# foolwood/SiamMask

Hardware: AMD Instinct MI355X
Metric: frames/sec (255x255 search, 127x127 template) (higher is better)
Workload: dtype f16

## Files before the change

siammask_amd/csrc/conv_plan.h:

```cpp
#pragma once
#include <string>
#include <vector>

#include "smk_kernels.h"

struct Act {
    void *p = nullptr;
    int H = 0, W = 0, C = 0;
};

struct PackedConv {
    void *w = nullptr;
    void *w_halo = nullptr;
    void *w_frag = nullptr;
    void *w_frag_halo = nullptr;
    void *w_frag16 = nullptr;
    float *bias = nullptr;
    int N = 0;
    int rows = 0;
    int group_rows = 0;
    int groups = 1;
    int Ci = 0, k = 1, K = 0, Kpad = 0;
    int kw = 0;
    int alg_k = 0;
// ... 2 lines not shown
    bool x3 = false;
};

struct ConvOpt {
    int stride = 1, pad = 0, dil = 1, relu = 0;
    int stride_x = 0;
    const Act *res = nullptr;
    int res_mode = smk::RES_NONE;
    int res_coff = 0;
    int cin_off = 0;
    int cout_off = 0;
    int n_override = 0;
    int groups = 1;
    bool win = false;
    int Hl = 0, Wl = 0, org_y = 0, org_x = 0;
    const int *pos = nullptr;
    int pos_mul = 0, pos_add = 0;
    bool ups = false;
    float *nchw_out = nullptr;
    int algo_naive = 0;
    int tile_code = 0;
    int halo = 0;
    int wreg = 0;
};

inline int kdtype(int dtype) { return dtype == smk::DT_F16X3 ? smk::DT_F16 : dtype; }
inline const char *dtname(int dt) { return dt == smk::DT_F16 ? "f16" : "f32"; }

#pragma GCC visibility push(hidden)

enum ConvKernel { CK_NAIVE, CK_IGEMM, CK_HALO, CK_WREG, CK_PP };
struct ConvPlan {
    int kind = CK_IGEMM;
    smk::TileChoice tile{};
    int halo_bm = 0;
    int wreg = 0;
    int stages = 0;
};

extern const int WREG_TILE[9][2];

smk::TileChoice tile_from_code(int code, const smk::ConvParams &p, int dtype);
int halo_choice(const PackedConv &pc, const smk::ConvParams &p, const ConvOpt &o, int dtype);
int wreg_choice(const smk::ConvParams &p, const ConvOpt &o, int dtype, long ncu);
int wreg_stages(int ctx_dtype, int B);
int wreg_stages_from_code(int code);
// ... 28 lines not shown
```

siammask_amd/csrc/conv_wreg.hip:

```cpp
#include <hip/hip_runtime.h>
#include <type_traits>
#include "smk_kernels.h"

namespace smk {

#include "wreg_tile.inc"

template <int WK, int MODE> struct WregDepth {
    static constexpr int NSTAGE = MODE == 8 ? 2 * WK + 1 : MODE;
    static constexpr int WT = MODE == 8 ? 2 * WK : 2;
};

template <int FM, int WN, int WK, int MODE, int NPW>
__global__ __launch_bounds__((WN * WK + NPW) * 64, ((NPW == 2 && WregLds<FM, WregDepth<WK, MODE>::NSTAGE, WN * WK>::v <= 80 * 1024) ? 2 : 1))
void conv_wreg_kernel(const ConvBatch cb) {
    constexpr int NSTAGE = WregDepth<WK, MODE>::NSTAGE, WT = WregDepth<WK, MODE>::WT;
    int pi = 0;
#pragma unroll
    for (int i = 1; i < CONV_BATCH_MAX; ++i)
        if (i < cb.n && (int)blockIdx.x >= cb.start[i]) pi = i;
    const ConvParams &p = cb.p[pi];
    set_wave_prio(cb.p[0].wave_prio);
    const int wg_first = cb.start[pi], wg_count = cb.start[pi + 1] - cb.start[pi];
    constexpr int BM = 32 * FM, BN = 64 * WN;
    __shared__ __attribute__((aligned(16))) unsigned char smem[WregLds<FM, NSTAGE, WN * WK>::v];
    const int tilesN = (p.Nst + BN - 1) / BN;
    int t = (int)blockIdx.x - wg_first;
    if (p.xcd_mode != 0) {
        const int nblk = wg_count, q = nblk >> 3, r = nblk & 7;
        const int x = t & 7, j = t >> 3;
        t = x * q + (x < r ? x : r) + j;
    }
    const int tm = t / tilesN, tn = t - tm * tilesN;
    wreg_tile<FM, WN, WK, NSTAGE, 0, WT, NPW>(p, (int)blockIdx.z, tm * BM, p.M, tn * BN, smem);
}

#ifdef SMK_MEASURE
template <int FM, int WN, int WK, int ABL>
__global__ __launch_bounds__(512, 1)
void conv_wreg_ablate_kernel(const ConvBatch cb) {
    const ConvParams &p = cb.p[0];
    constexpr int BM = 32 * FM, BN = 64 * WN;
    __shared__ __attribute__((aligned(16))) unsigned char smem[WregLds<FM, 3>::v];
    const int tilesN = (p.Nst + BN - 1) / BN;
    const int t = (int)blockIdx.x;
    const int tm = t / tilesN, tn = t - tm * tilesN;
    wreg_tile<FM, WN, WK, 3, (ABL << 8), 2, 4>(p, 0, tm * BM, p.M, tn * BN, smem);
}
#endif

template <int FM, int WN, int WK>
static int launch_wreg_t(ConvBatch &cb, int stages, hipStream_t s) {
    constexpr int BM = 32 * FM, BN = 64 * WN;
    int total = 0, groups = 1;
    for (int i = 0; i < cb.n; ++i) {
        ConvParams &p = cb.p[i];
        cb.start[i] = total;
        total += ((p.M + BM - 1) / BM) * ((p.Nst + BN - 1) / BN);
        if (p.groups > groups) groups = p.groups;
        p.ksplit = 1;
        if (p.x3_ct > 0 && p.x3_in > 0) {
            p.Ci = p.x3_in * X3_PLANES;
            p.ci_shift = -1;
            for (int sh = 0; sh < 16; ++sh)
                if ((1 << sh) == p.Ci) p.ci_shift = sh;
            p.x3_in = 0;
        }
    }
    for (int i = cb.n; i <= CONV_BATCH_MAX; ++i) cb.start[i] = total;
    dim3 grid(total, 1, groups);
#ifdef SMK_MEASURE
    if constexpr ((WN == 2 && WK == 2) || (WN == 4 && WK == 1))
    if (g_tune.ablate && cb.n == 1 && groups == 1) {
        switch (g_tune.ablate) {
        case 1: hipLaunchKernelGGL((conv_wreg_ablate_kernel<FM, WN, WK, 1>), grid, dim3(512), 0, s, cb); break;
        case 2: hipLaunchKernelGGL((conv_wreg_ablate_kernel<FM, WN, WK, 2>), grid, dim3(512), 0, s, cb); break;
        case 3: hipLaunchKernelGGL((conv_wreg_ablate_kernel<FM, WN, WK, 3>), grid, dim3(512), 0, s, cb); break;
        case 4: hipLaunchKernelGGL((conv_wreg_ablate_kernel<FM, WN, WK, 4>), grid, dim3(512), 0, s, cb); break;
        case 7: hipLaunchKernelGGL((conv_wreg_ablate_kernel<FM, WN, WK, 7>), grid, dim3(512), 0, s, cb); break;
        case 8: hipLaunchKernelGGL((conv_wreg_ablate_kernel<FM, WN, WK, 8>), grid, dim3(512), 0, s, cb); break;
        case 16: hipLaunchKernelGGL((conv_wreg_ablate_kernel<FM, WN, WK, 16>), grid, dim3(512), 0, s, cb); break;
        case 32: hipLaunchKernelGGL((conv_wreg_ablate_kernel<FM, WN, WK, 32>), grid, dim3(512), 0, s, cb); break;
        case 64: hipLaunchKernelGGL((conv_wreg_ablate_kernel<FM, WN, WK, 64>), grid, dim3(512), 0, s, cb); break;
        case 11: hipLaunchKernelGGL((conv_wreg_ablate_kernel<FM, WN, WK, 11>), grid, dim3(512), 0, s, cb); break;
        case 27: hipLaunchKernelGGL((conv_wreg_ablate_kernel<FM, WN, WK, 27>), grid, dim3(512), 0, s, cb); break;
        default: hipLaunchKernelGGL((conv_wreg_ablate_kernel<FM, WN, WK, 23>), grid, dim3(512), 0, s, cb); break;
        }
        return hipGetLastError() == hipSuccess ? 0 : -4;
    }
#endif
    if (g_tune.npw == 4) {
#ifdef SMK_MEASURE
        if (stages == 8 && WK > 1) {
            hipLaunchKernelGGL((conv_wreg_kernel<FM, WN, WK, (WK > 1 ? 8 : 3), 4>), grid, dim3((WN * WK + 4) * 64), 0, s, cb);
            return hipGetLastError() == hipSuccess ? 0 : -4;
        }
        if (stages == 5 || stages == 6 || stages == 7) {
            if (stages == 5) hipLaunchKernelGGL((conv_wreg_kernel<FM, WN, WK, 5, 4>), grid, dim3((WN * WK + 4) * 64), 0, s, cb);
            else if (stages == 6) hipLaunchKernelGGL((conv_wreg_kernel<FM, WN, WK, 6, 4>), grid, dim3((WN * WK + 4) * 64), 0, s, cb);
            else hipLaunchKernelGGL((conv_wreg_kernel<FM, WN, WK, 7, 4>), grid, dim3((WN * WK + 4) * 64), 0, s, cb);
            return hipGetLastError() == hipSuccess ? 0 : -4;
        }
#endif
        if (stages == 4) hipLaunchKernelGGL((conv_wreg_kernel<FM, WN, WK, 4, 4>), grid, dim3((WN * WK + 4) * 64), 0, s, cb);
        else hipLaunchKernelGGL((conv_wreg_kernel<FM, WN, WK, 3, 4>), grid, dim3((WN * WK + 4) * 64), 0, s, cb);
    } else {
        if (stages == 4) hipLaunchKernelGGL((conv_wreg_kernel<FM, WN, WK, 4, 2>), grid, dim3((WN * WK + 2) * 64), 0, s, cb);
        else hipLaunchKernelGGL((conv_wreg_kernel<FM, WN, WK, 3, 2>), grid, dim3((WN * WK + 2) * 64), 0, s, cb);
    }
    return hipGetLastError() == hipSuccess ? 0 : -4;
}

bool conv_wreg_eligible(const ConvParams &p, int dtype) {
    return dtype == DT_F16 && p.out_mode == OUT_NHWC && p.wgt_frag != nullptr && p.buf_lds && (p.Kpad % 128) == 0 &&
           (p.groups <= 1 || (p.g_wgt_off % 32) == 0);
}

int launch_conv_wreg_batch(ConvBatch &cb, int bm, int bn, int stages, void *stream) {
    hipStream_t s = (hipStream_t)stream;
    if (cb.n < 1 || cb.n > CONV_BATCH_MAX) return -1;
    for (int i = 0; i < cb.n; ++i)
        if (!conv_wreg_eligible(cb.p[i], DT_F16) || (cb.p[i].groups > 1) != (cb.p[0].groups > 1)) return 1;
    if (bm == 32) {
        if (bn == 64) return launch_wreg_t<1, 1, 4>(cb, stages, s);
    } else if (bm == 64) {
        if (bn == 256) return launch_wreg_t<2, 4, 1>(cb, stages, s);
        if (bn == 128) return launch_wreg_t<2, 2, 2>(cb, stages, s);
        if (bn == 64) return launch_wreg_t<2, 1, 4>(cb, stages, s);
    } else if (bm == 96) {
        if (bn == 256) return launch_wreg_t<3, 4, 1>(cb, stages, s);
    } else if (bm == 128) {
        if (bn == 256) return launch_wreg_t<4, 4, 1>(cb, stages, s);
        if (bn == 128) return launch_wreg_t<4, 2, 2>(cb, stages, s);
        if (bn == 64) return launch_wreg_t<4, 1, 4>(cb, stages, s);
    }
    return 1;
}

// ... 2 lines not shown
```

siammask_amd/csrc/engine.cpp:

```cpp
#include <hip/hip_runtime_api.h>

#include <cmath>
#include <cstdarg>
#include <tuple>
#include <cstdio>
#include <cstdlib>
#include <cstring>
#include <functional>
#include <map>
#include <memory>
#include <string>
#include <vector>

#include "../../include/siammask_hip.h"
#include "../../include/siammask_hip_test.h"
#include "conv_plan.h"
#include "smk_kernels.h"
#include "tracker_state.h"
#include "vot_overlap.h"

using namespace smk;

static thread_local std::string g_err;

// ... 717 lines not shown
        if (!out) return fail(SMK_E_ARG, "conv without output");
        if (out->H != p.Ho || out->W != p.Wo)
            return fail(SMK_E_ARG, "internal: conv output %dx%d != buffer %dx%d", p.Ho, p.Wo, out->H, out->W);
        p.out = out->p;
        p.out_mode = OUT_NHWC;
        p.Cos = out->C;
        p.cout_off = o.cout_off;
        p.Nst = rup(p.N, 8);
        if (pc.x3) {
            p.x3_out = o.groups > 1 ? pc.group_rows : out->C / X3_PLANES;
            if (out->C % X3_PLANES || o.cout_off + (o.groups - 1) * X3_PLANES * pc.group_rows + p.x3_out + p.Nst > out->C)
                return fail(SMK_E_ARG, "internal: split conv output channels exceed buffer");
        } else if (o.cout_off + (o.groups - 1) * pc.group_rows + p.Nst > out->C)
            return fail(SMK_E_ARG, "internal: conv output channels exceed buffer");
    }
    p.xcd_mode = g_tune.xcd_mode;
    if (o.nchw_out && g_tune.nchw_tn_major && p.xcd_mode == 1 && p.M >= 20000 && (double)p.M * p.N * 4 >= 4.0e6) p.xcd_mode = 2;
    p.prio = g_tune.prio;
    p.wave_prio = env.wave_prio;
    {
        const double ib = (double)B * in.H * in.W * in.C * esize(env.dtype), wb = (double)pc.rows * pc.Kpad * esize(env.dtype);
        p.buf_lds = (g_tune.buf_lds && ib < 2.0e9 && wb < 2.0e9) ? 1 : 0;
        p.a_stage = g_tune.a_stage;
        p.res_nt = g_tune.res_nt;
        p.in_bytes = (unsigned)(ib < 4.0e9 ? ib : 0);
        p.w_bytes = (unsigned)(wb < 4.0e9 ? wb : 0);
    }
    p.nt_store = (g_tune.nt_store && o.nchw_out && (double)p.M * p.N * 4 >= 4.0e6) ? 1 : 0;
    p.ci_shift = -1;
    for (int sh = 0; sh < 16; ++sh)
        if ((1 << sh) == p.Ci) p.ci_shift = sh;
    p.kw_magic = 65536 / p.kw + 1;
    p.zero = env.device >= 0 ? zero_page() : nullptr;
    if (env.device >= 0 && !p.zero) return fail(SMK_E_HIP, "could not allocate the zero page");
    if (o.res) {
        p.res = o.res->p;
        p.res_Cs = o.res->C;
        p.res_coff = o.res_coff;
        p.res_mode = o.res_mode;
        if (pc.x3) p.x3_res = o.res->C / X3_PLANES;
    }
    p.ksplit = 1;
    p.ks_part = env.ks_part;
    p.ks_cnt = env.ks_cnt;
    p.ks_part_cap = env.ks_part ? KS_PART_FLOATS : 0;
    p.ks_cnt_cap = env.ks_cnt ? KS_CNT : 0;
// ... 423 lines not shown
                    paired = run_conv_pair(c, (id + "c3").c_str(), t2, out, o3, "adjust", se, oa0, B, s);
                    if (paired < 0) return paired;
                    if (paired == 0) adjust_done = true;
                }
            }
            if (paired == 1) CHK(run_conv(c, (id + "c3").c_str(), t2, &out, B, o3, s, &rec));
            cur = out;
            sp = so;
        }
    }
    ConvOpt oa;
    if (sp < 20) {
        Act zf = ACT(c, T_ZF, sp - 8, sp - 8);
        oa.win = true; oa.Hl = oa.Wl = sp - 8; oa.org_y = oa.org_x = 4;
        CHK(run_conv(c, "adjust", cur, &zf, B, oa, s, &rec));
    } else if (!adjust_done) {
        Act se = ACT(c, T_SEARCH, sp, sp);
        CHK(run_conv(c, "adjust", cur, &se, B, oa, s, &rec));
    }
    if (c->seq_on && search_nb > 0 && sp >= 20 && g_tune.seq_search && c->seq.rec.size() < (size_t)SEQ_MAX) {
        Act se = ACT(c, T_SEARCH, sp, sp);
        Act xs = ACT(c, T_XS, sp - 2, sp - 2);
        ConvOpt o; o.relu = 1; o.n_override = 256 * search_nb;
        CHK(run_conv(c, "conv_search", se, &xs, B, o, s, &rec));
        if (search_done) *search_done = true;
    }
    if (c->seq_on) CHK(seq_flush(c, rec, B, s));
    c->last_B = B; c->last_S = S;
    return 0;
}

static int seq_template(smk_ctx *c, StepRec &rec, const float *z, int B, hipStream_t s) {
    CHK(run_backbone(c, rec, z, B, 127, s));
    Act zf = ACT(c, T_ZF);
    Act zk = ACT(c, T_ZK);
    ConvOpt o; o.relu = 1;
    CHK(run_conv(c, "conv_kernel", zf, &zk, B, o, s));
    return 0;
}

static int mask_head_args(smk_ctx *c, float *mask, Act &h0, ConvOpt &om) {
    CHK(act(h0, c, T_HEAD0));
    om.nchw_out = mask;
    om.cin_off = branch_off(c, 2);
    return 0;
}

static int seq_track(smk_ctx *c, StepRec &rec, const float *x, int B, int flags, float *cls, float *loc, float *mask,
                     hipStream_t s, int phase = PH_ALL) {
    const bool x3 = c->dtype == DT_F16X3;
    const int nbt = nbranch(c);
    const int nb = (flags & SMK_TRACK_MASK) ? nbt : 2;
    bool search_done = false;
    CHK(run_backbone(c, rec, x, B, 255, s, phase, nb, &search_done));
    Act se = ACT(c, T_SEARCH);
    Act xs = ACT(c, T_XS);
    ConvOpt o; o.relu = 1; o.n_override = 256 * nb;
    if (!search_done) CHK(run_conv(c, "conv_search", se, &xs, B, o, s));
    if (rec.gate_late) {
        if (launch_pipe_gate(c->pipe_cnt, c->seq_err, c->seq_err_hdev, s, 0, nullptr, c->pipe_cnt + 8)) return fail(SMK_E_HIP, "pipe_gate launch failed");
        rec.has_seq = true;
    }
    Act zk = ACT(c, T_ZK);
    Act corr = ACT(c, T_CORR);
    Act h0 = ACT(c, T_HEAD0);
    const bool want_mask = (flags & SMK_TRACK_MASK) && !(flags & SMK_TRACK_NO_MASK_HEAD);
    bool fused_heads = false;
    if (c->dtype == DT_F16 && g_tune.corr_head) {
        auto ih = c->conv.find("head0"), ic = c->conv.find("cls3"), il = c->conv.find("loc3");
        if (ih != c->conv.end() && ic != c->conv.end() && il != c->conv.end() && ih->second.w_frag && ic->second.w_frag && il->second.w_frag &&
            ih->second.Kpad == 256 && ic->second.Kpad == 256 && il->second.Kpad == 256 && ih->second.group_rows == 256 &&
            ic->second.N == 10 && il->second.N == 20) {
            CorrHeadParams hp;
            memset(&hp, 0, sizeof(hp));
            hp.xs = (const _Float16 *)xs.p; hp.zk = (const _Float16 *)zk.p; hp.corr = (_Float16 *)corr.p; hp.h0 = (_Float16 *)h0.p;
            hp.w0_frag = ih->second.w_frag; hp.b0 = ih->second.bias; hp.w0_bytes = (unsigned)((size_t)ih->second.rows * ih->second.Kpad * 2);
            hp.w3_frag[0] = ic->second.w_frag; hp.b3[0] = ic->second.bias; hp.out3[0] = cls; hp.n3[0] = 10;
            hp.w3_frag[1] = il->second.w_frag; hp.b3[1] = il->second.bias; hp.out3[1] = loc; hp.n3[1] = 20;
            hp.w3_bytes[0] = (unsigned)((size_t)ic->second.rows * ic->second.Kpad * 2);
            hp.w3_bytes[1] = (unsigned)((size_t)il->second.rows * il->second.Kpad * 2);
// ... 29 lines not shown
            const ConvParams &mp = rec.deferred_mask.p;
            rec.deferred_mask.flop = 2.0 * mp.M * (double)mp.N * mp.kh * mp.kw * mp.Ci;
            rec.deferred_mask.bytes = (double)mp.M * mp.Ci * esize(c->dtype) + (double)mp.M * mp.N * 4 + (double)mp.N * mp.Ci * esize(c->dtype);
            rec.deferred_mask.have = true;
        } else {
            CHK(run_conv(c, "mask3", hm, nullptr, B, om, s));
        }
    }
    c->last_nb = nb;
    return 0;
}

static bool refine_splittable(const smk_ctx *c, int B) {
    return kdtype(c->dtype) == DT_F16 && g_tune.chain && g_tune.merge && (g_tune.merge == 2 || B <= g_tune.merge_max_batch);
}
static int seq_refine(smk_ctx *c, StepRec &rec, int B, float *out, hipStream_t s, int part = 0) {
    const int *pos = c->pos_dev;
    Act corr = ACT(c, T_CORR);
    Act p0 = ACT(c, T_P0), p1 = ACT(c, T_P1), p2 = ACT(c, T_P2);
    ConvOpt r3; r3.pad = 1; r3.relu = 1;
    ConvOpt w2 = r3; w2.win = true; w2.Hl = w2.Wl = 15; w2.pos = pos; w2.pos_mul = 1; w2.pos_add = -4;
    ConvOpt w1 = r3; w1.win = true; w1.Hl = w1.Wl = 31; w1.pos = pos; w1.pos_mul = 2; w1.pos_add = -8;
    ConvOpt w0 = r3; w0.win = true; w0.Hl = w0.Wl = 61; w0.pos = pos; w0.pos_mul = 4; w0.pos_add = -16;
    Act d = ACT(c, T_RF_D);
    Act d1 = d;
    d1.H = d1.W = 1; d1.C = d.H * d.W * d.C;
    ConvOpt od; od.win = true; od.Hl = od.Wl = 1; od.pos = pos; od.pos_mul = 1; od.cin_off = branch_off(c, 2);
    Act v2a = ACT(c, T_RF_V2A), v1a = ACT(c, T_RF_V1A), v0a = ACT(c, T_RF_V0A);
    const bool merged = (!c->prof || c->prof_merge) && g_tune.merge && (g_tune.merge == 2 || B <= g_tune.merge_max_batch);
    if (merged && part != 2) {
        w2.tile_code = 4;
        if (g_tune.rf_wreg & 1) w2.wreg = w1.wreg = w0.wreg = od.wreg = ((g_tune.rf_wreg >> 4) & 15) ? ((g_tune.rf_wreg >> 4) & 15) : 3;
        CHK(run_conv_jobs(c, {{"v2.0", &p2, &v2a, w2}, {"v1.0", &p1, &v1a, w1}, {"v0.0", &p0, &v0a, w0},
                              {"deconv", &corr, &d1, od}}, B, 0, s));
    } else if (part != 2) {
        CHK(run_conv(c, "deconv", corr, &d1, B, od, s));
    }
    if (kdtype(c->dtype) == DT_F16 && g_tune.chain) {
        if (!merged && part != 2) {
            CHK(run_conv(c, "v2.0", p2, &v2a, B, w2, s));
            CHK(run_conv(c, "v1.0", p1, &v1a, B, w1, s));
            CHK(run_conv(c, "v0.0", p0, &v0a, B, w0, s));
        }
        Act V2 = ACT(c, T_RF_S2), V1 = ACT(c, T_RF_S1), V0 = ACT(c, T_RF_S0);
        ConvOpt r3l = r3;
        r3l.tile_code = g_tune.rf_tile2;
// ... 1142 lines not shown
        in.C *= X3_PLANES;
    }
    std::vector<float> fused;
    if (x3 && g_tune.x3_fused && fuse_rows_x3(rows, pc, g->k * g->k, pc.Ci / 3, fused)) CHK(upload_packed(pc, rows, bias, dtype, &fused));
    else
    CHK(upload_packed(pc, rows, bias, dtype));
    TmpBufs tmp;
    tmp.v.push_back(pc.w); tmp.v.push_back(pc.bias);
    if (pc.w_frag) tmp.v.push_back(pc.w_frag);
    if (pc.w_frag16) tmp.v.push_back(pc.w_frag16);
    if (pc.oscale) tmp.v.push_back(pc.oscale);
    const size_t es = esize(dtype);
    CHK(tmp.alloc(&in.p, (size_t)g->B * g->H * g->W * in.C * es));
    CvtInParams ci{x_dev, in.p, g->B, g->Cin, g->H, g->W, x3 ? in.C / X3_PLANES : in.C, 0, x3 ? 1 : 0};
    if (x3 ? launch_cvt_in_x3(ci, s) : launch_cvt_in(ci, dtype, s)) return fail(SMK_E_HIP, "cvt_in launch failed");
    int *pos_dev = nullptr;
    if (pos_host) {
        CHK(tmp.alloc((void **)&pos_dev, sizeof(int) * 2 * g->B));
        HIPCHK(hipMemcpyAsync(pos_dev, pos_host, sizeof(int) * 2 * g->B, hipMemcpyHostToDevice, s));
        o.pos = pos_dev;
    }
    const int mode = algo & 0xff;
    const bool nchw = (mode == 2 || mode == 3);
    if (mode == 4) {
        CHK(upload_halo_pack(pc, rows, dtype));
        if (pc.w_frag_halo) tmp.v.push_back(pc.w_frag_halo);
        if (pc.w_halo) tmp.v.push_back(pc.w_halo);
    }
    Act out, res;
    out.H = Ho; out.W = Wo; out.C = rup(g->Cout, 8) * (x3 ? X3_PLANES : 1);
    if (res_dev && g->res_mode) {
        if (nchw) return fail(SMK_E_ARG, "residual is not supported with the NCHW epilogue");
        res = out;
        CHK(tmp.alloc(&res.p, (size_t)g->B * Ho * Wo * out.C * es));
        CvtInParams cr{res_dev, res.p, g->B, g->Cout, Ho, Wo, x3 ? out.C / X3_PLANES : out.C, 0, x3 ? 1 : 0};
        if (x3 ? launch_cvt_in_x3(cr, s) : launch_cvt_in(cr, dtype, s)) return fail(SMK_E_HIP, "cvt_in launch failed");
        o.res = &res; o.res_mode = g->res_mode;
    }
    ConvEnv env;
    env.dtype = ctx_dtype;
    HIPCHK(hipGetDevice(&env.device));
    CHK(op_ks_scratch(env));
    ConvParams p;
    if (nchw) {
        o.nchw_out = y_dev;
        CHK(conv_params(env, pc, in, nullptr, g->B, o, p));
// ... 970 lines not shown
```

siammask_amd/csrc/smk_kernels.h:

```cpp
#pragma once
#include <stdint.h>

#if defined(__HIPCC__)
#define SMK_HD __host__ __device__ inline
#else
#define SMK_HD inline
#endif

namespace smk {

enum { DT_F32 = 0, DT_F16 = 1, DT_F16X3 = 2 };
enum { RES_NONE = 0, RES_PRE_RELU = 1, RES_POST_RELU = 2 };
enum { OUT_NHWC = 0, OUT_NCHW_F32 = 1 };

constexpr int NPAD_ALIGN = 128;
constexpr int KPAD_ALIGN = 128;

struct ConvParams {
    const void *in;
    const void *wgt;
    const void *wgt_frag;
    const void *wgt_frag_halo;
    const float *bias;
    const void *res;
// ... 10 lines not shown
    int ups;
    int Ho, Wo;
    int kh, kw, stride, pad, dil;
    int stride_x;
    int K, Kpad;
    int N;
    int Nst;
    int M;
    int Cos, cout_off;
    int res_Cs, res_coff;
    int relu, res_mode, out_mode;
    int groups;
    int g_cin_off;
    int g_wgt_off;
    int g_cout_off;
    int xcd_mode;
    int ci_shift;
    int kw_magic;
    int prio;
    int wave_prio;
    int buf_lds;
    int a_stage;
    int res_nt;
    unsigned in_bytes, w_bytes;
    int nt_store;
    int x3_out, x3_res, x3_in;
    int x3_ct, x3_nreal;
    const float *oscale;
    int ksplit;
    float *ks_part;
    unsigned *ks_cnt;
    size_t ks_part_cap;
    int ks_cnt_cap;
};

constexpr int CONV_BATCH_MAX = 4;
struct ConvBatch {
    int n;
    int start[CONV_BATCH_MAX + 1];
    ConvParams p[CONV_BATCH_MAX];
};

struct SeqLayer {
    const void *in;
    const void *wgt_frag;
    const float *bias;
    const void *res;
    void *out;
    unsigned in_bytes, w_bytes;
    int kw_magic;
    unsigned short Hs, Ws, Hl, Wl, Ho, Wo, Cs, cin_off, Ci, Kpad, Nst, Cos, res_Cs, res_coff, cout_off, bar_ord;
    short org_y, org_x;
    signed char kh, kw, stride, stride_x, pad, dil, relu, res_mode, ci_shift;
    signed char cfg;
    signed char sync;
    signed char a_stage;
    signed char kstag;
// ... 14 lines not shown
constexpr int SEQ_CFG_C2C3C1_MID = 30;
constexpr int SEQ_XCH_SLAB = 32768;
constexpr int SEQ_XCH_PAIRS = 16;
constexpr size_t SEQ_XCH_BYTES = (size_t)8 * SEQ_XCH_PAIRS * 4 * SEQ_XCH_SLAB;
constexpr int SEQ_CFG_HALO128 = 24;
constexpr int SEQ_CFG_HALO64 = 25;
constexpr int SEQ_YRES_IN = 2, SEQ_YRES_NOSTORE = 4, SEQ_LDS_HI = 8;
constexpr int SEQ_YRES_BYTES = 65536;
constexpr int SEQ_MAX = 36;
struct SeqArgs {
    int n, B;
    int flags, pad_;
    unsigned *bar;
    float *xch;
    int *err;
    int *err_host;
    unsigned long long *clk;
    unsigned long long *clk2;
    unsigned *exit_sem;
    SeqLayer L[SEQ_MAX];
};
static_assert(sizeof(SeqArgs) <= 4096, "the layer list travels in the kernel-argument segment");

struct Tuning {
    int xcd_mode = 1;
    int force_tile = 0;
    int min_blocks_x16 = 16;
    int stages = 0;
    int kt = 0;
    int prio = 0;
    int nt_store = 1;
    int halo = 1;
    int halo_db = 1;
    int chain = 1;
    int ksplit = 0;
    int xc_ch = 64;
    int l1_fused = 1;
    int stem_fused = 1;
    int xc_full = 0;
    int buf_lds = 1;
    int chain_mask = 1;
    int nchw_tn_major = 1;
    int merge = 1;
    int merge_max_batch = 32;
    int rf_wreg = 3;
    int seq_fuse3 = 0;
// ... 157 lines not shown
    float *out;
    int H, W, model_sz;
    int box[CROP_MAX_B][3];
    unsigned char avg[CROP_MAX_B][4];
};
struct PasteParams {
    const float *logits;
    unsigned char *mask_out;
    float *prob_out;
    int ms, W, H;
    float seg_thr, border;
    double inv_map[CROP_MAX_B][6];
};

struct TileChoice { int bm, bn, kt, stages; };
TileChoice choose_tile(const ConvParams &p, int dtype);
int launch_conv_mfma(const ConvParams &p, int dtype, TileChoice t, void *stream);
int launch_conv_mfma_batch(ConvBatch &cb, int dtype, TileChoice t, void *stream);
int launch_conv_naive(const ConvParams &p, int dtype, void *stream);
int conv_ksplit(const ConvParams &p, int dtype, const TileChoice &t);
__attribute__((visibility("hidden"))) bool conv_halo_eligible(const ConvParams &p, int dtype, int bm);
int launch_conv_halo(const ConvParams &p, int dtype, int bm, void *stream);
bool conv_wreg_eligible(const ConvParams &p, int dtype);
int launch_conv_wreg_batch(ConvBatch &cb, int bm, int bn, int stages, void *stream);
bool conv_pp_eligible(const ConvParams &p, int dtype);
int launch_conv_pp(const ConvParams &p, void *stream);
int launch_conv_seq(const SeqArgs &a, int grid, void *stream);
int launch_conv_pair(const SeqLayer &L3, const SeqLayer &L1, int code, int M, void *stream, int rows);
int conv_seq_occupancy();
int xcc_census(int grid, int *out_host);
struct RefineChainLayer {
    const void *w;
    const float *bias;
    int Kpad, Ci;
};
struct RefineChainParams {
    const void *d;
    const void *v2, *v1, *v0;
    int v2_cs, v1_cs, v0_cs;
    RefineChainLayer L[9];
    float *out;
    int B;
    unsigned long long *clk;
    _Float16 *ring;
    int *ring_cursor;
    unsigned *ring_done;
// ... 47 lines not shown
```

siammask_amd/csrc/wreg_tile.inc:

```

typedef _Float16 half8 __attribute__((ext_vector_type(8)));
typedef float floatx16 __attribute__((ext_vector_type(16)));
typedef float floatx4 __attribute__((ext_vector_type(4)));
typedef unsigned uint4v __attribute__((ext_vector_type(4)));
typedef __attribute__((address_space(3))) void lds_void_t;

template <int A, int B> struct WMax { static constexpr int v = A > B ? A : B; };

template <class P> __device__ __forceinline__ RowInfo row_info_t(const P &p, int m) {
    RowInfo r;
    const int hw = p.Ho * p.Wo;
    r.b = m / hw;
    const int rem = m - r.b * hw;
    const int oy = rem / p.Wo, ox = rem - oy * p.Wo;
    r.ly0 = oy * p.stride - p.pad;
    r.lx0 = ox * p.stride_x - p.pad;
    r.oy_org = p.org_y;
    r.ox_org = p.org_x;
    if (p.pos) {
        r.oy_org += p.pos[2 * r.b + 0] * p.pos_mul + p.pos_add;
        r.ox_org += p.pos[2 * r.b + 1] * p.pos_mul + p.pos_add;
    }
    return r;
}

template <int FM, int NSTAGE, int NCW = 4> struct WregLds {
    static constexpr int v = WMax<NSTAGE * 32 * FM * 128, NCW * 32 * FM * 68 * 4>::v;
};

struct NoHoist { __device__ __forceinline__ bool operator()() const { return true; } };

template <int FM, int WN, int WK, int NSTAGE, int AUX, int WT = 2, int NPW = 2, int CLK = 0, class P = ConvParams, class HOIST = NoHoist>
__device__ __forceinline__ bool wreg_tile(const P &p, const int g, const int m0, const int m_end, const int n0,
                                          unsigned char *smem, unsigned long long *tclk = nullptr, const int kt0 = 0,
                                          const HOIST hoist = HOIST()) {
    typedef _Float16 T;
    constexpr int NCW = WN * WK, NT = (NCW + NPW) * 64;
    static_assert(NPW == 2 || NPW == 4, "two or four producer waves");
    static_assert(NCW == 4 && (WK == 1 || WK == 2 || WK == 4), "four consumer waves");
    constexpr int BM = 32 * FM, BN = 64 * WN;
    constexpr int KT = 128, BK = 64, VE = 8;
    constexpr int RPR = NPW * 64 / 8;
    constexpr int RA = BM / RPR;
    constexpr int NKS = 4 / WK;
    constexpr int D = WT * NKS;
    static_assert(D % 2 == 0, "the A-fragment double buffer alternates with the parity of the step inside a macro-iteration");
    constexpr int AHEAD = NSTAGE - 1;
    constexpr int STAGE_BYTES = BM * KT;
    constexpr int LDE = 68;

    int tid = threadIdx.x;
    asm volatile("" : "+v"(tid));
    const int lane = tid & 63;
    const int wave = __builtin_amdgcn_readfirstlane(tid >> 6);
    auto stamp = [&](int i) {
        if constexpr (CLK != 0) {
            if (tclk && tid == 0) {
                tclk[i] = wall_clock64();
                if (i == 0) tclk[8] = __builtin_readcyclecounter();
                if (i == 6) tclk[9] = __builtin_readcyclecounter();
            }
        }
    };
    stamp(0);
    const int cout_off = p.cout_off + g * p.g_cout_off;
    const float *bias = p.bias + g * p.g_wgt_off;
    const int nk = p.Kpad / BK;
    auto rot = [&](int kt) { const int r = kt + kt0; return r >= nk ? r - nk : r; };
    const int x3ct = std::is_same<P, SeqLayer>::value ? 0 : __builtin_amdgcn_readfirstlane(p.x3_ct);
    const int nkp = x3ct > 0 ? __builtin_amdgcn_readfirstlane(p.x3_nreal) : nk;

    floatx16 acc[FM][2];

    if (wave >= NCW) {
        const int ptid = tid - NCW * 64, pw = wave - NCW;
        const int cin_off = p.cin_off + g * p.g_cin_off;
        const int lrow = ptid >> 3;
        const int wslot = (ptid & 7) ^ ((lrow >> 1) & 7);
        constexpr bool ASTAGE_OK = !std::is_same<P, SeqLayer>::value;
        const bool a_staged = ASTAGE_OK && p.a_stage && x3ct == 0;
        const int slot = a_staged ? (ptid & 7) : wslot;
        RowInfo ri[RA];
        bool rvalid[RA];
#pragma unroll
        for (int i = 0; i < RA; ++i) {
            const int m = m0 + lrow + RPR * i;
            rvalid[i] = m < m_end;
            ri[i] = row_info_t(p, rvalid[i] ? m : m0);
        }
        const __amdgpu_buffer_rsrc_t rs_in = __builtin_amdgcn_make_buffer_rsrc((void *)p.in, 0, p.in_bytes, 0x00020000);
        constexpr long OOB = 0x7ffff000;
        auto sgpr = [](int v) { return __builtin_amdgcn_readfirstlane(v); };
        int g_kwm = sgpr(p.kw_magic), g_kw = sgpr(p.kw), g_kh = sgpr(p.kh), g_dil = sgpr(p.dil), g_Hl = sgpr(p.Hl), g_Wl = sgpr(p.Wl),
            g_Hs = sgpr(p.Hs), g_Ws = sgpr(p.Ws), g_Cs = sgpr(p.Cs), g_cish = sgpr(p.ci_shift), g_Ci = sgpr(p.Ci);
        asm volatile("" : "+s"(g_kwm), "+s"(g_kw), "+s"(g_kh), "+s"(g_dil), "+s"(g_Hl), "+s"(g_Wl));
        asm volatile("" : "+s"(g_Hs), "+s"(g_Ws), "+s"(g_Cs), "+s"(g_cish), "+s"(g_Ci));
        const int g_x3in = std::is_same<P, SeqLayer>::value ? 0 : sgpr(p.x3_in);
// ... 94 lines not shown
        if (islot == NSTAGE) islot = 0;
        for (int kt = 0; kt < nkp; ++kt) {
            int younger = nkp - 1 - kt;
            if (younger > AHEAD - 1) younger = AHEAD - 1;
            static_assert(AHEAD >= 1 && AHEAD <= 8 && (AHEAD - 1) * RA < 64, "ring depth");
            constexpr int VM5 = AHEAD > 5 ? 5 * RA : 0, VM6 = AHEAD > 6 ? 6 * RA : 0, VM7 = AHEAD > 7 ? 7 * RA : 0;
            if (younger <= 0) asm volatile("s_waitcnt vmcnt(0)" ::: "memory");
            else if (younger == 1) asm volatile("s_waitcnt vmcnt(%0)" ::"n"(RA) : "memory");
            else if (younger == 2) asm volatile("s_waitcnt vmcnt(%0)" ::"n"(2 * RA) : "memory");
            else if (younger == 3) asm volatile("s_waitcnt vmcnt(%0)" ::"n"(3 * RA) : "memory");
            else if (younger == 4) asm volatile("s_waitcnt vmcnt(%0)" ::"n"(4 * RA) : "memory");
            else if (younger == 5) asm volatile("s_waitcnt vmcnt(%0)" ::"n"(VM5) : "memory");
            else if (younger == 6) asm volatile("s_waitcnt vmcnt(%0)" ::"n"(VM6) : "memory");
            else asm volatile("s_waitcnt vmcnt(%0)" ::"n"(VM7) : "memory");
            if (!(AUX & 0x800) || kt == 0) __builtin_amdgcn_s_barrier();
            asm volatile("" ::: "memory");
            if (kt + AHEAD < nkp && !(AUX & 0x100)) {
                set_tile(kt + AHEAD);
                issue_tile(islot);
            }
            if (++islot == NSTAGE) islot = 0;
        }
        }
    } else {
        const int wk = wave % WK, wn = wave / WK;
#pragma unroll
        for (int i = 0; i < FM; ++i)
#pragma unroll
            for (int j = 0; j < 2; ++j)
#pragma unroll
                for (int r = 0; r < 16; ++r) acc[i][j][r] = 0.f;
        const int frow = lane & 31, fhalf = lane >> 5;
        const int fsw = (frow >> 1) & 7;
        const int a_row_off = frow * KT;
        const int KS16 = p.Kpad >> 4;
        const __amdgpu_buffer_rsrc_t rs_w = __builtin_amdgcn_make_buffer_rsrc((void *)p.wgt_frag, 0, p.w_bytes, 0x00020000);
        const int nb0 = (g * p.g_wgt_off + n0) / 32 + wn * 2;
        const int wv0 = (nb0 * KS16) * 1024 + lane * 16;
        const int wv1 = wv0 + KS16 * 1024;
        half8 fa[2][FM], fb[D][2];
        if (AUX & 0x1000) {
#pragma unroll
            for (int h = 0; h < 2; ++h)
#pragma unroll
                for (int i = 0; i < FM; ++i)
#pragma unroll
                    for (int q = 0; q < 8; ++q) fa[h][i][q] = (_Float16)0.f;
        }
        auto load_w_half = [&](int gstep, int h, half8 &b) {
            const int kts = gstep / NKS, s = gstep - kts * NKS;
            const int so = (rot(kts) * 4 + s * WK + wk) * 1024;
            b = __builtin_bit_cast(half8, __builtin_amdgcn_raw_buffer_load_b128(rs_w, h ? wv1 : wv0, so, 0));
        };
        auto load_w = [&](int gstep, half8 (&b)[2]) {
            load_w_half(gstep, 0, b[0]);
            load_w_half(gstep, 1, b[1]);
        };
        auto read_a1 = [&](int buf, int s, int i, half8 &a) {
            if (AUX & 0x1000) {
                asm volatile("" : "+v"(a));
                return;
            }
            const int so = (((s * WK + wk) * 2 + fhalf) ^ fsw) << 4;
            a = *(const half8 *)(smem + buf * STAGE_BYTES + a_row_off + i * (32 * KT) + so);
        };
        auto read_a = [&](int buf, int s, half8 (&a)[FM]) {
#pragma unroll
            for (int i = 0; i < FM; ++i) read_a1(buf, s, i, a[i]);
        };
        auto mma1 = [&](const half8 &a, const half8 &b, floatx16 &c) {
            if (AUX & 0x400) {
                asm volatile("" ::"v"(a), "v"(b));
                return;
            }
            c = __builtin_amdgcn_mfma_f32_32x32x16_f16(a, b, c, 0, 0, 0);
        };
        auto mma_part = [&](const half8 (&a)[FM], const half8 (&b)[2], int q0, int q1) {
#pragma unroll
            for (int q = q0; q < q1; ++q) mma1(a[q >> 1], b[q & 1], acc[q >> 1][q & 1]);
        };
        const int S = nk * NKS;
#pragma unroll
        for (int j = 0; j < D; ++j)
// ... 28 lines not shown
                            if (!(AUX & 0x800)) __builtin_amdgcn_s_barrier();
                            asm volatile("" ::: "memory");
                            cur = nxt;
                            read_a(cur, 0, fa[(j + 1) & 1]);
                        }
                        __builtin_amdgcn_sched_barrier(0);
                        mma_part(fa[j & 1], fb[j], FM, 2 * FM);
                        __builtin_amdgcn_sched_barrier(0);
                    }
                    if (do_refill) load_w(g0 + j + D, fb[j]);
                } else {
                    const bool tile_end = s + 1 == NKS;
                    const bool more = !(decltype(last)::value && j == (WT > 2 ? nsteps : D) - 1);
#pragma unroll
                    for (int i = 0; i < FM; ++i) {
                        mma1(fa[j & 1][i], fb[j][0], acc[i][0]);
                        __builtin_amdgcn_sched_barrier(0);
                        if (i == 0 && tile_end && more) {
                            bool adv = true;
                            if (x3ct > 0) {
                                if (++x3r == 3 * x3ct) x3r = 0;
                                adv = !(x3r < 2 * x3ct && (x3r & 1));
                            }
                            if (adv) {
                                int nxt = cur + 1;
                                if (nxt == NSTAGE) nxt = 0;
                                asm volatile("s_waitcnt lgkmcnt(0)" ::: "memory");
                                if (!(AUX & 0x800)) __builtin_amdgcn_s_barrier();
                                asm volatile("" ::: "memory");
                                cur = nxt;
                            }
                        }
                        if (more) read_a1(cur, tile_end ? 0 : s + 1, i, fa[(j + 1) & 1][i]);
                        __builtin_amdgcn_sched_barrier(0);
                    }
                    if (do_refill) load_w_half(g0 + j + D, 0, fb[j][0]);
                    __builtin_amdgcn_sched_barrier(0);
#pragma unroll
                    for (int i = 0; i < FM; ++i) {
                        mma1(fa[j & 1][i], fb[j][1], acc[i][1]);
                        __builtin_amdgcn_sched_barrier(0);
                    }
                    if (do_refill) load_w_half(g0 + j + D, 1, fb[j][1]);
                    __builtin_amdgcn_sched_barrier(0);
                }
            }
        };
// ... 98 lines not shown
```

siammask_amd/ops.py:

```python
import ctypes

import numpy as np
import torch

from . import _lib

ALGO = {"mfma": 0, "naive": 1, "mfma_nchw": 2, "naive_nchw": 3, "halo": 4, "wreg": 5, "pp": 6}
WREG_TILE = {(64, 256): 1, (64, 128): 2, (64, 64): 3, (128, 256): 4, (128, 128): 5, (128, 64): 6, (96, 256): 7, (32, 64): 8}
TILE = {None: 0, "auto": 0, (128, 128): 1, (128, 64): 2, (64, 128): 3, (64, 64): 4, (256, 128): 5}


def _chk_cuda(*ts):
    for t in ts:
        if t is not None and not t.is_cuda:
            raise RuntimeError("siammask_amd.ops run on the MI355X only (got a CPU tensor)")


def tile_code(tile=None, kt=0, stages=0):
    return TILE[tile] | ({0: 0, 128: 1, 256: 2}[kt] << 4) | ({0: 0, 2: 1, 3: 2, 4: 3}[stages] << 6)


def wreg_code(tile, stages=0):
    return WREG_TILE[tuple(tile)] | ({0: 0, 8: 1, 3: 2, 4: 3}[stages] << 6)


def conv2d(x, w, b=None, stride=1, pad=0, dil=1, relu=False, res=None, res_mode=1, dtype="f32",
           algo="mfma", tile=None, win=None, ups=None, pos=None, pos_mul=0, pos_add=0, org=(0, 0),
           cin_off=0, cin_len=0, kt=0, stages=0):
    _chk_cuda(x, res)
    x = x.contiguous().float()
    B, Cin, H, W = x.shape
    w = np.ascontiguousarray(w.detach().cpu().numpy() if isinstance(w, torch.Tensor) else w, dtype=np.float32)
    bb = None if b is None else np.ascontiguousarray(
        b.detach().cpu().numpy() if isinstance(b, torch.Tensor) else b, dtype=np.float32)
    g = _lib.ConvGeom()
    g.B, g.Cin, g.H, g.W = B, Cin, H, W
    g.Cout, g.k, g.stride, g.pad, g.dil = w.shape[0], w.shape[2], stride, pad, dil
    g.relu = int(bool(relu))
    g.res_mode = res_mode if res is not None else 0
    g.cin_off, g.cin_len = cin_off, cin_len
    g.org_y, g.org_x = org
    g.pos_mul, g.pos_add = pos_mul, pos_add
    Hl, Wl = H, W
    if win is not None:
        g.win, g.Hl, g.Wl = 1, win[0], win[1]
        Hl, Wl = win
    if ups is not None:
        g.ups, g.Hl, g.Wl = 1, ups[0], ups[1]
        Hl, Wl = ups
    Ho = (Hl + 2 * pad - dil * (g.k - 1) - 1) // stride + 1
    Wo = (Wl + 2 * pad - dil * (g.k - 1) - 1) // stride + 1
    y = torch.empty((B, g.Cout, Ho, Wo), dtype=torch.float32, device=x.device)
    p = None if pos is None else np.ascontiguousarray(pos, dtype=np.int32)
    r = None if res is None else res.contiguous().float()
    code = ALGO[algo] | ((wreg_code(tile, stages) if algo == "wreg" else tile_code(tile, kt, stages)) << 8)
    vp = lambda a: a.ctypes.data_as(ctypes.c_void_p) if a is not None else None
    with torch.cuda.device(x.device):
        _lib.check(_lib.lib().smk_op_conv2d_ex(
            _lib.DTYPE[dtype], code, ctypes.byref(g), x.data_ptr(), vp(w), vp(bb),
            r.data_ptr() if r is not None else None, vp(p), y.data_ptr(), _lib.current_stream_ptr()))
    return y


SEQ_CFG = {None: -1, (64, 256): 0, (64, 128): 1, (64, 64): 2, (128, 256): 3, (128, 128): 4, "deep": 5,
           "no_a": 6, "no_w": 7, "no_mfma": 8, (128, 64): 9,
           "abl10": 10, "abl11": 11, "abl12": 12, "abl13": 13, "abl14": 14, "old64x128": 15, "old128x256": 16, "old64x256": 17, "old64x64": 18,
           "halo128": 24, "halo64": 25}


def seq_ops(x_shape, layers):
    B = x_shape[0]
    arr = (_lib.SeqOp * len(layers))()
    keep = []
    shapes = [tuple(x_shape[1:])]
    for i, l in enumerate(layers):
        w = np.ascontiguousarray(l["w"], dtype=np.float32)
        b = None if l.get("b") is None else np.ascontiguousarray(l["b"], dtype=np.float32)
        keep += [w, b]
# ... 142 lines not shown
```

Before: 14850.

## Add resident-patch wreg conv variant that stages the input halo in LDS once

Adds a wreg convolution path for 3x3 stride-1 f16 convs. The producer waves load the whole input patch (output rows plus a halo) into LDS once, and the consumer waves read the A fragments straight from that resident patch across all nine taps, with no per-K-step A staging. It is enabled through g_tune.rf_wreg bits for the search conv and the refine convs, and exposed via ops.py as resident=. The aim is to remove the repeated im2col-style global reads and the per-stage A pipeline sync, at the cost of large LDS use (up to 160KB), one block per CU, and a tile shape limited to whole output rows.

```diff
diff --git a/siammask_amd/csrc/conv_plan.h b/siammask_amd/csrc/conv_plan.h
--- a/siammask_amd/csrc/conv_plan.h
+++ b/siammask_amd/csrc/conv_plan.h
@@ -48,6 +48,7 @@
     int tile_code = 0;
     int halo = 0;
     int wreg = 0;
+    int a_res = 0;
 };
 
 inline int kdtype(int dtype) { return dtype == smk::DT_F16X3 ? smk::DT_F16 : dtype; }
diff --git a/siammask_amd/csrc/conv_wreg.hip b/siammask_amd/csrc/conv_wreg.hip
--- a/siammask_amd/csrc/conv_wreg.hip
+++ b/siammask_amd/csrc/conv_wreg.hip
@@ -35,6 +35,40 @@
     wreg_tile<FM, WN, WK, NSTAGE, 0, WT, NPW>(p, (int)blockIdx.z, tm * BM, p.M, tn * BN, smem);
 }
 
+template <int LB> struct WregResLds { static constexpr int v = LB ? 160 * 1024 : 80 * 1024; };
+template <int FM, int WN, int WK, int LB, int WTR>
+__global__ __launch_bounds__((WN * WK + 4) * 64, 1)
+void conv_wreg_res_kernel(const ConvBatch cb) {
+    constexpr int NSTAGE = 3;
+    static_assert(WregLds<FM, NSTAGE, WN * WK>::v <= WregResLds<LB>::v, "LDS");
+    int pi = 0;
+#pragma unroll
+    for (int i = 1; i < CONV_BATCH_MAX; ++i)
+        if (i < cb.n && (int)blockIdx.x >= cb.start[i]) pi = i;
+    const ConvParams &p = cb.p[pi];
+    set_wave_prio(cb.p[0].wave_prio);
+    const int wg_first = cb.start[pi], wg_count = cb.start[pi + 1] - cb.start[pi];
+    constexpr int BM = 32 * FM, BN = 64 * WN;
+    __shared__ __attribute__((aligned(16))) unsigned char smem[WregResLds<LB>::v];
+    const int tilesN = (p.Nst + BN - 1) / BN;
+    int t = (int)blockIdx.x - wg_first;
+    if (p.xcd_mode != 0) {
+        const int nblk = wg_count, q = nblk >> 3, r = nblk & 7;
+        const int x = t & 7, j = t >> 3;
+        t = x * q + (x < r ? x : r) + j;
+    }
+    const int tm = t / tilesN, tn = t - tm * tilesN;
+    if (p.a_res) {
+        const int rpt = BM / p.Wo, rtiles = (p.Ho + rpt - 1) / rpt, hw = p.Ho * p.Wo;
+        const int img = tm / rtiles, oy0 = (tm - img * rtiles) * rpt;
+        const int m0 = img * hw + oy0 * p.Wo;
+        const int m_end = min(m0 + rpt * p.Wo, (img + 1) * hw);
+        wreg_tile<FM, WN, WK, NSTAGE, 0, WTR, 4, 0, ConvParams, NoHoist, 1>(p, 0, m0, m_end, tn * BN, smem, nullptr, 0, NoHoist(), img, oy0);
+    } else {
+        wreg_tile<FM, WN, WK, NSTAGE, 0, 2, 4>(p, (int)blockIdx.z, tm * BM, p.M, tn * BN, smem);
+    }
+}
+
 #ifdef SMK_MEASURE
 template <int FM, int WN, int WK, int ABL>
 __global__ __launch_bounds__(512, 1)
@@ -52,10 +86,25 @@
 template <int FM, int WN, int WK>
 static int launch_wreg_t(ConvBatch &cb, int stages, hipStream_t s) {
     constexpr int BM = 32 * FM, BN = 64 * WN;
-    int total = 0, groups = 1;
+    constexpr bool RES_TILE = (FM == 3 && WN == 4 && WK == 1) || (WN == 1 && WK == 4 && (FM == 1 || FM == 2));
+    constexpr int RES_LDS_MAX = FM == 1 ? WregResLds<0>::v : WregResLds<1>::v;
+    int total = 0, groups = 1, res_lds = 0;
     for (int i = 0; i < cb.n; ++i) {
         ConvParams &p = cb.p[i];
         cb.start[i] = total;
+        const int want = p.a_res;
+        p.a_res = 0;
+        if (want > 0) {
+            const bool ok = RES_TILE && stages == 3 && g_tune.npw == 4 && !g_tune.ablate && conv_wreg_res_eligible(p, BM) &&
+                            wreg_res_geom(p, BM).bytes <= RES_LDS_MAX;
+            if (!ok && want == 2) return 1;
+            p.a_res = ok ? 1 : 0;
+        }
+        if (p.a_res) {
+            const WregResGeom rg = wreg_res_geom(p, BM);
+            if (rg.bytes > res_lds) res_lds = rg.bytes;
+            total += (p.M / (p.Ho * p.Wo)) * rg.rtiles * ((p.Nst + BN - 1) / BN);
+        } else
         total += ((p.M + BM - 1) / BM) * ((p.Nst + BN - 1) / BN);
         if (p.groups > groups) groups = p.groups;
         p.ksplit = 1;
@@ -69,6 +118,17 @@
     }
     for (int i = cb.n; i <= CONV_BATCH_MAX; ++i) cb.start[i] = total;
     dim3 grid(total, 1, groups);
+    if constexpr (RES_TILE) {
+        if (res_lds > 0) {
+            constexpr int WTR = WK == 4 ? 4 : 2;
+            const dim3 blk((WN * WK + 4) * 64);
+            if (FM == 1 || (FM == 2 && res_lds <= WregResLds<0>::v))
+                hipLaunchKernelGGL((conv_wreg_res_kernel<FM, WN, WK, (FM == 3 ? 1 : 0), WTR>), grid, blk, 0, s, cb);
+            else
+                hipLaunchKernelGGL((conv_wreg_res_kernel<FM, WN, WK, (FM == 1 ? 0 : 1), WTR>), grid, blk, 0, s, cb);
+            return hipGetLastError() == hipSuccess ? 0 : -4;
+        }
+    }
 #ifdef SMK_MEASURE
     if constexpr ((WN == 2 && WK == 2) || (WN == 4 && WK == 1))
     if (g_tune.ablate && cb.n == 1 && groups == 1) {
@@ -114,6 +174,14 @@
 bool conv_wreg_eligible(const ConvParams &p, int dtype) {
     return dtype == DT_F16 && p.out_mode == OUT_NHWC && p.wgt_frag != nullptr && p.buf_lds && (p.Kpad % 128) == 0 &&
            (p.groups <= 1 || (p.g_wgt_off % 32) == 0);
+}
+
+bool conv_wreg_res_eligible(const ConvParams &p, int bm) {
+    if (!conv_wreg_eligible(p, DT_F16) || p.kh != 3 || p.kw != 3 || p.stride != 1 || p.stride_x != 1 || p.dil != 1 || p.groups > 1 || p.ups) return false;
+    if (p.Ci < 64 || p.Ci % 64 || p.K != 9 * p.Ci || p.x3_ct || p.x3_in || p.pad < 0 || p.Wo < 1 || p.Wo > bm || p.Ho < 1) return false;
+    if (p.M % (p.Ho * p.Wo)) return false;
+    const WregResGeom g = wreg_res_geom(p, bm);
+    return g.npieces < 65536 && g.PW < 65536 && g.bytes <= 160 * 1024;
 }
 
 int launch_conv_wreg_batch(ConvBatch &cb, int bm, int bn, int stages, void *stream) {
diff --git a/siammask_amd/csrc/engine.cpp b/siammask_amd/csrc/engine.cpp
--- a/siammask_amd/csrc/engine.cpp
+++ b/siammask_amd/csrc/engine.cpp
@@ -763,6 +763,7 @@
         const double ib = (double)B * in.H * in.W * in.C * esize(env.dtype), wb = (double)pc.rows * pc.Kpad * esize(env.dtype);
         p.buf_lds = (g_tune.buf_lds && ib < 2.0e9 && wb < 2.0e9) ? 1 : 0;
         p.a_stage = g_tune.a_stage;
+        p.a_res = o.a_res;
         p.res_nt = g_tune.res_nt;
         p.in_bytes = (unsigned)(ib < 4.0e9 ? ib : 0);
         p.w_bytes = (unsigned)(wb < 4.0e9 ? wb : 0);
@@ -1232,6 +1233,7 @@
         Act se = ACT(c, T_SEARCH, sp, sp);
         Act xs = ACT(c, T_XS, sp - 2, sp - 2);
         ConvOpt o; o.relu = 1; o.n_override = 256 * search_nb;
+        o.a_res = (c->dtype == DT_F16 && (g_tune.rf_wreg & WREG_RES_SEARCH)) ? 1 : 0;
         CHK(run_conv(c, "conv_search", se, &xs, B, o, s, &rec));
         if (search_done) *search_done = true;
     }
@@ -1266,6 +1268,7 @@
     Act se = ACT(c, T_SEARCH);
     Act xs = ACT(c, T_XS);
     ConvOpt o; o.relu = 1; o.n_override = 256 * nb;
+    o.a_res = (c->dtype == DT_F16 && (g_tune.rf_wreg & WREG_RES_SEARCH)) ? 1 : 0;
     if (!search_done) CHK(run_conv(c, "conv_search", se, &xs, B, o, s));
     if (rec.gate_late) {
         if (launch_pipe_gate(c->pipe_cnt, c->seq_err, c->seq_err_hdev, s, 0, nullptr, c->pipe_cnt + 8)) return fail(SMK_E_HIP, "pipe_gate launch failed");
@@ -1341,6 +1344,9 @@
     ConvOpt w2 = r3; w2.win = true; w2.Hl = w2.Wl = 15; w2.pos = pos; w2.pos_mul = 1; w2.pos_add = -4;
     ConvOpt w1 = r3; w1.win = true; w1.Hl = w1.Wl = 31; w1.pos = pos; w1.pos_mul = 2; w1.pos_add = -8;
     ConvOpt w0 = r3; w0.win = true; w0.Hl = w0.Wl = 61; w0.pos = pos; w0.pos_mul = 4; w0.pos_add = -16;
+    if (c->dtype == DT_F16) {
+        w1.a_res = (g_tune.rf_wreg & WREG_RES_V1) ? 1 : 0; w2.a_res = (g_tune.rf_wreg & WREG_RES_V2) ? 1 : 0; w0.a_res = (g_tune.rf_wreg & WREG_RES_V0) ? 1 : 0;
+    }
     Act d = ACT(c, T_RF_D);
     Act d1 = d;
     d1.H = d1.W = 1; d1.C = d.H * d.W * d.C;
@@ -2529,6 +2535,7 @@
     }
     const int mode = algo & 0xff;
     const bool nchw = (mode == 2 || mode == 3);
+    if (mode == 5 && ((algo >> 12) & 3) == 1) o.a_res = 2;
     if (mode == 4) {
         CHK(upload_halo_pack(pc, rows, dtype));
         if (pc.w_frag_halo) tmp.v.push_back(pc.w_frag_halo);
diff --git a/siammask_amd/csrc/smk_kernels.h b/siammask_amd/csrc/smk_kernels.h
--- a/siammask_amd/csrc/smk_kernels.h
+++ b/siammask_amd/csrc/smk_kernels.h
@@ -56,6 +56,7 @@
     int buf_lds;
     int a_stage;
     int res_nt;
+    int a_res;
     unsigned in_bytes, w_bytes;
     int nt_store;
     int x3_out, x3_res, x3_in;
@@ -67,6 +68,21 @@
     size_t ks_part_cap;
     int ks_cnt_cap;
 };
+
+struct WregResGeom { int rpt, rtiles, PW, PR, pp, pitch, npieces, rounds, bytes; };
+SMK_HD WregResGeom wreg_res_geom(const ConvParams &p, int bm) {
+    WregResGeom g;
+    g.rpt = p.Wo > 0 && p.Wo <= bm ? bm / p.Wo : 0;
+    g.rtiles = g.rpt ? (p.Ho + g.rpt - 1) / g.rpt : 0;
+    g.PW = p.Wl + 2 * p.pad;
+    g.PR = (g.rpt + 2) * g.PW;
+    g.pp = p.Ci / 8 + 1;
+    g.pitch = g.pp * 16;
+    g.npieces = (g.PR + 1) * g.pp;
+    g.rounds = (g.npieces + 255) / 256;
+    g.bytes = g.rounds * 4096;
+    return g;
+}
 
 constexpr int CONV_BATCH_MAX = 4;
 struct ConvBatch {
@@ -127,6 +143,7 @@
 };
 static_assert(sizeof(SeqArgs) <= 4096, "the layer list travels in the kernel-argument segment");
 
+constexpr int WREG_RES_SEARCH = 1 << 12, WREG_RES_V1 = 1 << 13, WREG_RES_V2 = 1 << 14, WREG_RES_V0 = 1 << 15;
 struct Tuning {
     int xcd_mode = 1;
     int force_tile = 0;
@@ -330,6 +347,7 @@
 __attribute__((visibility("hidden"))) bool conv_halo_eligible(const ConvParams &p, int dtype, int bm);
 int launch_conv_halo(const ConvParams &p, int dtype, int bm, void *stream);
 bool conv_wreg_eligible(const ConvParams &p, int dtype);
+bool conv_wreg_res_eligible(const ConvParams &p, int bm);
 int launch_conv_wreg_batch(ConvBatch &cb, int bm, int bn, int stages, void *stream);
 bool conv_pp_eligible(const ConvParams &p, int dtype);
 int launch_conv_pp(const ConvParams &p, void *stream);
diff --git a/siammask_amd/csrc/wreg_tile.inc b/siammask_amd/csrc/wreg_tile.inc
--- a/siammask_amd/csrc/wreg_tile.inc
+++ b/siammask_amd/csrc/wreg_tile.inc
@@ -30,11 +30,12 @@
 
 struct NoHoist { __device__ __forceinline__ bool operator()() const { return true; } };
 
-template <int FM, int WN, int WK, int NSTAGE, int AUX, int WT = 2, int NPW = 2, int CLK = 0, class P = ConvParams, class HOIST = NoHoist>
+template <int FM, int WN, int WK, int NSTAGE, int AUX, int WT = 2, int NPW = 2, int CLK = 0, class P = ConvParams, class HOIST = NoHoist, int RES = 0>
 __device__ __forceinline__ bool wreg_tile(const P &p, const int g, const int m0, const int m_end, const int n0,
                                           unsigned char *smem, unsigned long long *tclk = nullptr, const int kt0 = 0,
-                                          const HOIST hoist = HOIST()) {
+                                          const HOIST hoist = HOIST(), const int res_img = 0, const int res_oy0 = 0) {
     typedef _Float16 T;
+    static_assert(RES == 0 || (AUX == 0 && NPW == 4 && !std::is_same<P, SeqLayer>::value), "resident patch: conv_wreg_kernel, four producer waves");
     constexpr int NCW = WN * WK, NT = (NCW + NPW) * 64;
     static_assert(NPW == 2 || NPW == 4, "two or four producer waves");
     static_assert(NCW == 4 && (WK == 1 || WK == 2 || WK == 4), "four consumer waves");
@@ -72,7 +73,41 @@
 
     floatx16 acc[FM][2];
 
-    if (wave >= NCW) {
+    if constexpr (RES != 0) {
+        if (wave >= NCW) {
+            const int ptid = tid - NCW * 64, pw = wave - NCW;
+            auto sgpr = [](int v) { return __builtin_amdgcn_readfirstlane(v); };
+            const __amdgpu_buffer_rsrc_t rs_in = __builtin_amdgcn_make_buffer_rsrc((void *)p.in, 0, p.in_bytes, 0x00020000);
+            constexpr int OOB = 0x7ffff000;
+            const int g_Hl = sgpr(p.Hl), g_Wl = sgpr(p.Wl), g_Hs = sgpr(p.Hs), g_Ws = sgpr(p.Ws), g_Cs = sgpr(p.Cs), g_pad = sgpr(p.pad);
+            const int PW = g_Wl + 2 * g_pad, PR = (BM / sgpr(p.Wo) + 2) * PW, PP = (sgpr(p.Ci) >> 3) + 1;
+            const unsigned mPP = 0xffffffffu / (unsigned)PP + 1u, mPW = 0xffffffffu / (unsigned)PW + 1u;
+            const int NR = ((PR + 1) * PP + NPW * 64 - 1) / (NPW * 64);
+            int oy_org = sgpr(p.org_y), ox_org = sgpr(p.org_x);
+            if (p.pos) {
+                oy_org += sgpr(p.pos[2 * res_img + 0]) * p.pos_mul + p.pos_add;
+                ox_org += sgpr(p.pos[2 * res_img + 1]) * p.pos_mul + p.pos_add;
+            }
+            const int ly0 = res_oy0 - g_pad;
+            const int base = (res_img * g_Hs + oy_org) * g_Ws + ox_org;
+            if (!hoist()) return false;
+            for (int j = 0; j < NR; ++j) {
+                const int q = j * (NPW * 64) + ptid;
+                const int pix = (int)__umulhi((unsigned)q, mPP), piece = q - pix * PP;
+                const int py = (int)__umulhi((unsigned)pix, mPW), px = pix - py * PW;
+                const int ly = ly0 + py, lx = px - g_pad;
+                const int sy = ly + oy_org, sx = lx + ox_org;
+                const bool ok = (piece < PP - 1) & (pix < PR) & ((unsigned)ly < (unsigned)g_Hl) & ((unsigned)lx < (unsigned)g_Wl) &
+                                ((unsigned)sy < (unsigned)g_Hs) & ((unsigned)sx < (unsigned)g_Ws);
+                const long off = ((long)(base + ly * g_Ws + lx) * g_Cs + p.cin_off) * (long)sizeof(T) + piece * 16;
+                __builtin_amdgcn_raw_ptr_buffer_load_lds(rs_in, (lds_void_t *)(smem + j * (NPW * 1024) + pw * 1024), 16, ok ? (int)off : OOB, 0, 0, 0);
+            }
+            asm volatile("s_waitcnt vmcnt(0)" ::: "memory");
+            __builtin_amdgcn_s_barrier();
+            asm volatile("" ::: "memory");
+        }
+    }
+    if (RES == 0 && wave >= NCW) {
         const int ptid = tid - NCW * 64, pw = wave - NCW;
         const int cin_off = p.cin_off + g * p.g_cin_off;
         const int lrow = ptid >> 3;
@@ -213,7 +248,7 @@
             if (++islot == NSTAGE) islot = 0;
         }
         }
-    } else {
+    } else if (RES == 0 || wave < NCW) {
         const int wk = wave % WK, wn = wave / WK;
 #pragma unroll
         for (int i = 0; i < FM; ++i)
@@ -224,6 +259,36 @@
         const int frow = lane & 31, fhalf = lane >> 5;
         const int fsw = (frow >> 1) & 7;
         const int a_row_off = frow * KT;
+        int r_arow[RES ? FM : 1], r_koff = 0, r_c = 0, r_kw = 0, r_kh = 0, r_trow = 0, r_Ci = 0, r_pitch = 0, r_PWp = 0, r_zero = 0;
+        if constexpr (RES != 0) {
+            const int Wo = __builtin_amdgcn_readfirstlane(p.Wo), PW = __builtin_amdgcn_readfirstlane(p.Wl + 2 * p.pad);
+            r_Ci = __builtin_amdgcn_readfirstlane(p.Ci);
+            r_pitch = 2 * r_Ci + 16;
+            r_PWp = PW * r_pitch;
+            const int npx = m_end - m0;
+            const int lane_off = fhalf * 16 + wk * 32;
+            r_zero = (BM / Wo + 2) * r_PWp + lane_off;
+#pragma unroll
+            for (int i = 0; i < FM; ++i) {
+                const int r = i * 32 + frow;
+                const int ry = r < npx ? r / Wo : 0, rx = r < npx ? r - ry * Wo : 0;
+                r_arow[i] = (ry * PW + rx) * r_pitch + lane_off;
+            }
+        }
+        auto res_advance = [&]() {
+            r_c += BK;
+            if (r_c == r_Ci) {
+                r_c = 0;
+                if (++r_kw == 3) { r_kw = 0; ++r_kh; r_trow += r_PWp; }
+            }
+            r_koff = r_trow + r_kw * r_pitch + 2 * r_c;
+            if (r_kh == 3 && r_kw == 0 && r_c == 0) {
+#pragma unroll
+                for (int i = 0; i < (RES ? FM : 1); ++i) r_arow[i] = r_zero;
+                r_trow = 0;
+            }
+            if (r_kh >= 3) r_koff = 2 * r_c;
+        };
         const int KS16 = p.Kpad >> 4;
         const __amdgpu_buffer_rsrc_t rs_w = __builtin_amdgcn_make_buffer_rsrc((void *)p.wgt_frag, 0, p.w_bytes, 0x00020000);
         const int nb0 = (g * p.g_wgt_off + n0) / 32 + wn * 2;
@@ -250,6 +315,10 @@
         auto read_a1 = [&](int buf, int s, int i, half8 &a) {
             if (AUX & 0x1000) {
                 asm volatile("" : "+v"(a));
+                return;
+            }
+            if constexpr (RES != 0) {
+                a = *(const half8 *)(smem + (r_arow[i] + r_koff) + s * (WK * 32));
                 return;
             }
             const int so = (((s * WK + wk) * 2 + fhalf) ^ fsw) << 4;
@@ -324,7 +393,9 @@
                                 if (++x3r == 3 * x3ct) x3r = 0;
                                 adv = !(x3r < 2 * x3ct && (x3r & 1));
                             }
-                            if (adv) {
+                            if constexpr (RES != 0) {
+                                res_advance();
+                            } else if (adv) {
                                 int nxt = cur + 1;
                                 if (nxt == NSTAGE) nxt = 0;
                                 asm volatile("s_waitcnt lgkmcnt(0)" ::: "memory");
diff --git a/siammask_amd/ops.py b/siammask_amd/ops.py
--- a/siammask_amd/ops.py
+++ b/siammask_amd/ops.py
@@ -20,13 +20,13 @@
     return TILE[tile] | ({0: 0, 128: 1, 256: 2}[kt] << 4) | ({0: 0, 2: 1, 3: 2, 4: 3}[stages] << 6)
 
 
-def wreg_code(tile, stages=0):
-    return WREG_TILE[tuple(tile)] | ({0: 0, 8: 1, 3: 2, 4: 3}[stages] << 6)
+def wreg_code(tile, stages=0, resident=None):
+    return WREG_TILE[tuple(tile)] | ({0: 0, 8: 1, 3: 2, 4: 3}[stages] << 6) | ({None: 0, True: 1, False: 2}[resident] << 4)
 
 
 def conv2d(x, w, b=None, stride=1, pad=0, dil=1, relu=False, res=None, res_mode=1, dtype="f32",
            algo="mfma", tile=None, win=None, ups=None, pos=None, pos_mul=0, pos_add=0, org=(0, 0),
-           cin_off=0, cin_len=0, kt=0, stages=0):
+           cin_off=0, cin_len=0, kt=0, stages=0, resident=None):
     _chk_cuda(x, res)
     x = x.contiguous().float()
     B, Cin, H, W = x.shape
@@ -53,7 +53,9 @@
     y = torch.empty((B, g.Cout, Ho, Wo), dtype=torch.float32, device=x.device)
     p = None if pos is None else np.ascontiguousarray(pos, dtype=np.int32)
     r = None if res is None else res.contiguous().float()
-    code = ALGO[algo] | ((wreg_code(tile, stages) if algo == "wreg" else tile_code(tile, kt, stages)) << 8)
+    if resident is not None and algo != "wreg":
+        raise ValueError("resident= is a property of algo='wreg'")
+    code = ALGO[algo] | ((wreg_code(tile, stages, resident) if algo == "wreg" else tile_code(tile, kt, stages)) << 8)
     vp = lambda a: a.ctypes.data_as(ctypes.c_void_p) if a is not None else None
     with torch.cuda.device(x.device):
         _lib.check(_lib.lib().smk_op_conv2d_ex(
```

After: 14500. -2.4%, worse.
